# danbider/gp-quadrature

Hardware: AMD Instinct MI355X
Metric: GP-fits/sec (fit + posterior mean at the N training points), N=1e6 d=2 SE kernel (higher is better)
Workload: dtype f64; 1 GPU; 2D squared-exponential l=0.2 var=2 sigma2=0.2, eps=1e-4, global N=1e6 synthetic (BASELINE configs[1] at the metric's N=1e6), points sharded over the GPUs; n_per_gpu=1000000, global_n=1000000, d=2, mtot=23, M=529, mean_cg_iters=68, parallelism=points sharded over 1 GPU(s), CG replicated

## Files before the change

gp-quadrature_amd/csrc/cg_persistent.hip:

```cpp
#include <cmath>
#include <cstdlib>

#include "cg_plan_host.hpp"
#include "common.hpp"
#include "spectral_weights.hpp"
#include "toeplitz_cg.hpp"

namespace efgp {

namespace pcg {

constexpr int kRedWaves = kThreads / 64;

struct Pass {
    int dim;
    int n;
    int nstages;
    int radix[6];
    int w1_log2;
    int lines_log2;
    int other[2];
    int lo[2], hi[2];
    int in_limit;
    int out_lo, out_hi;
    int vs_pos, vs_c0, vs_c1;
    int pstride, s0, s1;
    int tw_lds;
    const double2* tw_glob;
};

struct Geom {
    int d;
    int n[3];
    int F[3];
    int ld[3];
    int M;
    int padded;
    int npass;
    Pass fwd[3];
    Pass inv[3];
    const double2* tw[3];
    int tw_lds_off[3];
    int tw_lds_total;
    int fuse_mid;
};

struct Args {
    Geom g;
    const double2* ws;
    const double* diag;
    const double* diag_scale;
    int b_times_ws;
    int zero_x0;
    const double2* x0;
    const double2* vhat;
    double sigmasq;
    int variant;
    double tol;
    int early_stop;
    int batched;
    int max_iter;
    const double2* b;
    double2* x;
    int* iters;
    double* hist;
    int hist_cap;
    int lz_steps;
    double* lz_alpha;
    double* lz_beta;
    double* lz_norm2;
    int wk_kind, wk_mtot;
    double wk_nu, wk_ell, wk_c0, wk_h;
    double2* ws_out;
    const double2* vsrc;
    int vL0, vL1;
    double2* vhat_out;
#ifdef EFGP_CG_STAMPS
    long long* stamps;
#endif
};

#ifdef EFGP_CG_STAMPS
#define EFGP_STAMP(slot)                                                     \
    do {                                                                     \
        if (blockIdx.x == 0 && threadIdx.x == 0) {                           \
            const long long now__ = (long long)__builtin_readcyclecounter(); \
            a.stamps[slot] += now__ - stamp_prev;                            \
            stamp_prev = now__;                                              \
        }                                                                    \
    } while (0)
#else
#define EFGP_STAMP(slot) \
    do {                 \
    } while (0)
#endif

__device__ __forceinline__ double2 cmulp(double2 a, double2 b) {
    return make_double2(a.x * b.x - a.y * b.y, a.x * b.y + a.y * b.x);
}
__device__ __forceinline__ double2 cadd(double2 a, double2 b) { return make_double2(a.x + b.x, a.y + b.y); }
__device__ __forceinline__ double2 csub(double2 a, double2 b) { return make_double2(a.x - b.x, a.y - b.y); }
__device__ __forceinline__ double2 mul_mi(double2 a) { return make_double2(a.y, -a.x); }

template <int R>
__device__ __forceinline__ void dft_fwd(double2 (&v)[R]);

template <>
__device__ __forceinline__ void dft_fwd<2>(double2 (&v)[2]) {
    double2 a = v[0], b = v[1];
    v[0] = cadd(a, b);
    v[1] = csub(a, b);
}

template <>
__device__ __forceinline__ void dft_fwd<4>(double2 (&v)[4]) {
    double2 t0 = cadd(v[0], v[2]), t1 = csub(v[0], v[2]);
    double2 t2 = cadd(v[1], v[3]), t3 = mul_mi(csub(v[1], v[3]));
    v[0] = cadd(t0, t2);
    v[1] = cadd(t1, t3);
    v[2] = csub(t0, t2);
    v[3] = csub(t1, t3);
}

template <>
__device__ __forceinline__ void dft_fwd<8>(double2 (&v)[8]) {
    double2 e[4] = {v[0], v[2], v[4], v[6]};
    double2 o[4] = {v[1], v[3], v[5], v[7]};
    dft_fwd<4>(e);
    dft_fwd<4>(o);
    const double h = 0.70710678118654752440;
    double2 o1 = make_double2(h * (o[1].x + o[1].y), h * (o[1].y - o[1].x));
    double2 o2 = mul_mi(o[2]);
    double2 o3 = make_double2(h * (o[3].y - o[3].x), -h * (o[3].x + o[3].y));
    v[0] = cadd(e[0], o[0]);
    v[4] = csub(e[0], o[0]);
    v[1] = cadd(e[1], o1);
    v[5] = csub(e[1], o1);
    v[2] = cadd(e[2], o2);
    v[6] = csub(e[2], o2);
    v[3] = cadd(e[3], o3);
    v[7] = csub(e[3], o3);
}

struct V8 {
    double2 a0, a1, a2, a3, a4, a5, a6, a7;
};
template <int T>
__device__ __forceinline__ double2& v8(V8& v) {
    if constexpr (T == 0) return v.a0;
    else if constexpr (T == 1) return v.a1;
    else if constexpr (T == 2) return v.a2;
    else if constexpr (T == 3) return v.a3;
    else if constexpr (T == 4) return v.a4;
    else if constexpr (T == 5) return v.a5;
    else if constexpr (T == 6) return v.a6;
    else return v.a7;
}
template <int T, int R>
__device__ __forceinline__ void spectral_mul_regs(double2 (&v)[R], V8& sp) {
    if constexpr (T < R) {
        double2 val = cmulp(v[T], v8<T>(sp));
        val.y = -val.y;
        v[T] = val;
        spectral_mul_regs<T + 1, R>(v, sp);
    }
}
template <int T, int R>
__device__ __forceinline__ void spectral_load_regs(V8& sp, const double2* __restrict__ vhat, int idx0, int step) {
    if constexpr (T < R) {
        v8<T>(sp) = vhat[idx0 + T * step];
        spectral_load_regs<T + 1, R>(sp, vhat, idx0, step);
    }
}

template <int R, bool INV, bool MID>
__device__ __forceinline__ void stage(const Geom& g, const Pass& p, int Ns, int ns_log2, bool first, bool last,
// ... 881 lines not shown
    if (!(asym <= 1e-16 * bb) || ws_bad != 0.0) {
#pragma unroll
        for (int s = 0; s < KS; ++s) {
            if (ok[s]) {
                a.x[base + idx[s]] = make_double2(__builtin_nan(""), __builtin_nan(""));
                a.x[base + (M - 1 - idx[s])] = make_double2(__builtin_nan(""), __builtin_nan(""));
            }
        }
        if (tid == 0) a.iters[row] = -2;
        return;
    }
    const double bn = sqrt(bb);
    const double den = bn > 0.0 ? bn : 1.0;
    const double den_eps = den + 1e-16, rcp_den = 1.0 / den_eps;
    if (wave == 3 && lane == 0) s_rcp = 1.0 / (rz + 1e-16);
    int it = 0;
    for (; it < a.max_iter;) {
        apply_A(pv, Ap);
        if (stop) break;
        double pAp = 0.0;
#pragma unroll
        for (int s = 0; s < KS; ++s) pAp += pv[s].x * Ap[s].x + pv[s].y * Ap[s].y;
        pAp = block_sum_h(pAp * wgt, red) + 1e-16;
        EFGP_STAMP(3);
        const double alpha = rz / pAp;
        double rr = 0.0, rzn = 0.0;
        double2 zv[KS];
#pragma unroll
        for (int s = 0; s < KS; ++s) {
            xv[s].x += alpha * pv[s].x;
            xv[s].y += alpha * pv[s].y;
            rv[s].x -= alpha * Ap[s].x;
            rv[s].y -= alpha * Ap[s].y;
            zv[s] = precond ? make_double2(div_rcp(rv[s].x, dg[s], rdg[s]), div_rcp(rv[s].y, dg[s], rdg[s])) : rv[s];
            rr += rv[s].x * rv[s].x + rv[s].y * rv[s].y;
            rzn += rv[s].x * zv[s].x + rv[s].y * zv[s].y;
        }
        rr *= wgt;
        rzn *= wgt;
        EFGP_STAMP(4);
        block_sum_pair_h(rr, rzn, red);
        EFGP_STAMP(5);
        ++it;
        if (wave == 3) {
            const double ratio = div_rcp(sqrt(rr), den_eps, rcp_den);
            const bool conv = a.early_stop && ((ratio < a.tol) || (a.batched && sqrt(rr) < 1e-12));
            if (lane == 0) {
                if (a.hist && row == 0 && it <= a.hist_cap) a.hist[it - 1] = ratio;
                s_stop = conv ? 1 : 0;
                s_rcp = 1.0 / (rzn + 1e-16);
            }
        }
        const double beta = div_rcp(rzn, rz + 1e-16, rcp_rz);
#pragma unroll
        for (int s = 0; s < KS; ++s) pv[s] = make_double2(zv[s].x + beta * pv[s].x, zv[s].y + beta * pv[s].y);
        rz = rzn;
    }
#pragma unroll
    for (int s = 0; s < KS; ++s) {
        if (ok[s]) {
            a.x[base + idx[s]] = xv[s];
            if (k0 > 0) a.x[base + (M - 1 - idx[s])] = s64::conjd(xv[s]);
        }
    }
    if (tid == 0) a.iters[row] = it;
}

namespace h48 {
constexpr int kThreadsH = 256, kWavesH = kThreadsH / 64;
constexpr int F = 48, HF = 24, NR = 12;
constexpr int LDR = 56;
constexpr int LT = 28;
constexpr int LX = 72;
constexpr int LQ = 82;
constexpr int G_ELEMS = NR * LDR, T_ELEMS = 2 * NR * LT, Q_ELEMS = HF * LQ;
static_assert(NR * LX <= Q_ELEMS, "the row lines' scratch aliases the column lines' scratch");
constexpr int kLdsElems = G_ELEMS + T_ELEMS + Q_ELEMS;
constexpr int ND = 4 * F;
constexpr int NC = 25;
constexpr int kReread = 8;
constexpr int LDV = 49;
constexpr int kLdsElemsDense = F * LDV + (kThreadsH / 8) * LX;
static_assert(2 * G_ELEMS + NR * LX <= kLdsElemsDense, "the iteration's G, Yh and row scratch alias the prologue's grid");

__device__ __forceinline__ void dft3(double2 b0, double2 b1, double2 b2, double2& x0, double2& x1, double2& x2) {
    const double s = 0.86602540378443864676;
    const double2 sm = cadd(b1, b2), df = csub(b1, b2);
    x0 = cadd(b0, sm);
    const double2 m = make_double2(fma(-0.5, sm.x, b0.x), fma(-0.5, sm.y, b0.y));
    x1 = make_double2(fma(s, df.y, m.x), fma(-s, df.x, m.y));
    x2 = make_double2(fma(-s, df.y, m.x), fma(s, df.x, m.y));
}
__device__ __forceinline__ void dft6(double2 (&v)[6]) {
    const double s = 0.86602540378443864676;
    double2 e0, e1, e2, o0, o1, o2;
    dft3(v[0], v[2], v[4], e0, e1, e2);
    dft3(v[1], v[3], v[5], o0, o1, o2);
    const double2 w1 = make_double2(fma(s, o1.y, 0.5 * o1.x), fma(-s, o1.x, 0.5 * o1.y));
    const double2 w2 = make_double2(fma(s, o2.y, -0.5 * o2.x), fma(-s, o2.x, -0.5 * o2.y));
    v[0] = cadd(e0, o0);
    v[3] = csub(e0, o0);
    v[1] = cadd(e1, w1);
    v[4] = csub(e1, w1);
    v[2] = cadd(e2, w2);
    v[5] = csub(e2, w2);
}
__device__ __forceinline__ void wave_sync() {
    __builtin_amdgcn_fence(__ATOMIC_ACQ_REL, "wavefront");
    __builtin_amdgcn_wave_barrier();
}
__device__ __forceinline__ void exchange_8to6(const double2 (&v)[8], double2 (&u)[6], bool writer, double2* __restrict__ wr,
                                              const double2* __restrict__ rd, const double2 (&tw)[5]) {
    wave_sync();
    if (writer) s64::store8_all<1>(wr, v);
    wave_sync();
#pragma unroll
    for (int t = 0; t < 6; ++t) u[t] = rd[9 * t];
#pragma unroll
    for (int t = 1; t < 6; ++t) u[t] = cmulp(u[t], tw[t - 1]);
    dft6(u);
}
__device__ __forceinline__ double exchange_8to6_norm(const double2 (&v)[8], double2 (&u)[6], bool writer, double2* __restrict__ wr,
                                                     const double2* __restrict__ rd, const double2 (&tw)[5], const double2 (&x)[4],
                                                     double scale) {
    wave_sync();
    if (writer) s64::store8_all<1>(wr, v);
    wave_sync();
#pragma unroll
    for (int t = 0; t < 6; ++t) u[t] = rd[9 * t];
    __builtin_amdgcn_sched_barrier(0);
    const double x01 = fma(x[0].x, x[0].x, x[0].y * x[0].y) + fma(x[1].x, x[1].x, x[1].y * x[1].y);
    const double x23 = fma(x[2].x, x[2].x, x[2].y * x[2].y) + fma(x[3].x, x[3].x, x[3].y * x[3].y);
    const double xx = scale * (x01 + x23);
    __builtin_amdgcn_sched_barrier(0);
#pragma unroll
    for (int t = 1; t < 6; ++t) u[t] = cmulp(u[t], tw[t - 1]);
    dft6(u);
    return xx;
}
__device__ __forceinline__ void exchange_6to8(double2 (&u)[6], double2 (&v)[8], double2* __restrict__ wr, const double2* __restrict__ rd,
                                              const double2 (&tw)[5]) {
#pragma unroll
    for (int t = 1; t < 6; ++t) u[t] = cmulp(u[t], tw[t - 1]);
    wave_sync();
#pragma unroll
    for (int t = 0; t < 6; ++t) wr[t] = u[t];
    wave_sync();
    s64::load8_all<9>(rd, v);
    h64::dft8_out4(v);
}

__device__ __forceinline__ double half_wave_sum(double v) {
    EFGP_DPP_ADD(v, 0x111, 0xF);
    EFGP_DPP_ADD(v, 0x112, 0xF);
    EFGP_DPP_ADD(v, 0x114, 0xF);
    EFGP_DPP_ADD(v, 0x118, 0xF);
    EFGP_DPP_ADD(v, 0x142, 0xA);
    const int lo = __builtin_amdgcn_readlane(__double2loint(v), 31);
    const int hi = __builtin_amdgcn_readlane(__double2hiint(v), 31);
    return __hiloint2double(hi, lo);
}

__device__ __forceinline__ double exchange_6to8_quot(double2 (&u)[6], double2 (&v)[8], double2* __restrict__ wr,
                                                     const double2* __restrict__ rd, const double2 (&tw)[5], double part, double num) {
#pragma unroll
    for (int t = 1; t < 6; ++t) u[t] = cmulp(u[t], tw[t - 1]);
// ... 56 lines not shown
        wave_sync();
#pragma unroll
        for (int t = 0; t < 6; ++t) wr[t] = u6[t];
        wave_sync();
        s64::load8_all<9>(rd, x8);
        dft_fwd<8>(x8);
        if (act && j < 6) {
#pragma unroll
            for (int t = 0; t < 8; ++t) buf[line * LD + j + 6 * t] = x8[t];
        }
    }
    __syncthreads();
#pragma unroll
    for (int ps = 0; ps < PASSES; ++ps) {
        const int line = slot + ps * SLOTS;
        const bool act = line < F;
#pragma unroll
        for (int t = 0; t < 6; ++t) u6[t] = act ? buf[(j + 8 * t) * LD + line] : make_double2(0.0, 0.0);
        dft6(u6);
#pragma unroll
        for (int t = 1; t < 6; ++t) u6[t] = cmulp(u6[t], tw[t - 1]);
        wave_sync();
#pragma unroll
        for (int t = 0; t < 6; ++t) wr[t] = u6[t];
        wave_sync();
        s64::load8_all<9>(rd, x8);
        dft_fwd<8>(x8);
        if (act && j < 6) {
#pragma unroll
            for (int t = 0; t < 8; ++t) {
                vhat[(j + 6 * t) * F + line] = x8[t];
                if (KEEP) buf[(j + 6 * t) * LD + line] = x8[t];
            }
        }
    }
}

template <int NT>
__device__ __forceinline__ void dense48_coeffs(double2* lds2, const double2 (&tw)[5], const double2* __restrict__ twg, int n,
                                               double2 (&cf)[NC]) {
    constexpr int SLOTS = NT / 8, PASSES = (F + SLOTS - 1) / SLOTS;
    double2* const buf = lds2;
    double2* const scr = lds2 + F * LDV;
    const int tid = threadIdx.x, slot = tid >> 3, j = tid & 7;
    double2* const wr = scr + slot * LX + 9 * j;
    const double2* const rd = scr + slot * LX + j;
    double2 u6[6], x8[8];
#pragma unroll
    for (int ps = 0; ps < PASSES; ++ps) {
        const int line = slot + ps * SLOTS;
        const bool act = line < F;
#pragma unroll
        for (int t = 0; t < 6; ++t) u6[t] = act ? s64::conjd(buf[(j + 8 * t) * LDV + line]) : make_double2(0.0, 0.0);
        dft6(u6);
#pragma unroll
        for (int t = 1; t < 6; ++t) u6[t] = cmulp(u6[t], tw[t - 1]);
        wave_sync();
#pragma unroll
        for (int t = 0; t < 6; ++t) wr[t] = u6[t];
        wave_sync();
        s64::load8_all<9>(rd, x8);
        dft_fwd<8>(x8);
        if (act && j < 6) {
#pragma unroll
            for (int t = 0; t < 8; ++t) buf[(j + 6 * t) * LDV + line] = s64::conjd(x8[t]);
        }
    }
    __syncthreads();
    const int f1 = tid % F, a0 = 3 * (tid / F);
    const bool dense = tid < ND;
    const double2 wc = twg[((n - 1) * f1) % F];
#pragma unroll
    for (int i = 0; i < NC; ++i) {
        const int l = a0 - 11 + i, al = l < 0 ? -l : l;
        double2 c = make_double2(0.0, 0.0);
        if (dense && al <= n - 1) {
            const double2 r = buf[(al + n - 1) * LDV + f1];
            c = make_double2(fma(r.y, wc.y, r.x * wc.x), fma(-r.x, wc.y, r.y * wc.x));
            if (l < 0) c.y = -c.y;
            if (l == 0) c.y = 0.0;
        }
        cf[i] = c;
    }
}
}

template <int VARIANT, bool FUSED = false, bool DENSE = true, bool FREQ_DOT = false>
__global__ __launch_bounds__(h48::kThreadsH) void cg_herm48_kernel(Args a) {
    using namespace h48;
    using h64::block_sum_h;
    using h64::block_sum_pair_h;
    using h64::dft8_in4;
    using h64::div_rcp;
    constexpr int KS = 4;
    static_assert(h64::kWavesH == kWavesH, "the block reductions are shared with the 64 x 64 kernel");
    static_assert(DENSE || !FREQ_DOT, "the row-frequency <p,Ap> reads what the per-frequency Toeplitz products hold");
    extern __shared__ double2 lds2[];
    __shared__ double red[4 * kWavesH];
    __shared__ double s_rcp;
    __shared__ int s_stop;
    __shared__ double s_part[FREQ_DOT ? ND + 8 * NR : 1];
    double2* const Gb = lds2;
    double2* const Tb = lds2 + G_ELEMS;
    double2* const Qb = Tb + (DENSE ? G_ELEMS : T_ELEMS);
    const int n = a.g.n[0], h = (n - 1) / 2, M = a.g.M;
    const int row = blockIdx.x;
    const int64_t base = (int64_t)row * M;
    const int tid = threadIdx.x, lane = tid & 63, wave = tid >> 6;
    const int k0 = tid >> 3, j = tid & 7;
    const bool row_role = tid < 8 * NR, vec_role = row_role && j < 6;
    const int jc = lane >> 3, ql = lane & 7, q = wave * 8 + ql;
    const bool col_role = wave < 3, col6 = jc < 6;
    const int k0s = row_role ? k0 : 0;
    double2* const xw = Qb + k0s * LX + 9 * j;
    const double2* const xr = Qb + k0s * LX + j;
    const int qs = col_role ? q : 0;
    double2* const qw = Qb + qs * LQ + 9 * jc;
    const double2* const qr = Qb + qs * LQ + jc;
    const bool dense_role = tid < ND;
    const int f1d = tid % F, kd = 3 * (tid / F);

    double2 twr[5], twc[5];
#pragma unroll
    for (int t = 1; t < 6; ++t) {
        twr[t - 1] = a.g.tw[0][j * t];
        twc[t - 1] = a.g.tw[0][jc * t];
    }
    if (FUSED) {
        vhat48_lines<kThreadsH, true>(a.vsrc, a.vL0, a.vL1, 1.0 / 2304.0, a.vhat_out, lds2);
        __syncthreads();
    }
    double sa[6], sb[6];
    double2 cf[DENSE ? NC : 1];
    if constexpr (DENSE) {
        if (!FUSED) {
#pragma unroll
            for (int k = 0; k < F * F / kThreadsH; ++k) {
                const int t = tid + k * kThreadsH, i0 = t / F, i1 = t - i0 * F;
                lds2[i0 * LDV + i1] = a.vhat[t];
            }
            __syncthreads();
        }
        dense48_coeffs<kThreadsH>(lds2, twr, a.g.tw[0], n, cf);
        __syncthreads();
    } else {
        const double2* const vh = FUSED ? lds2 : a.vhat;
        constexpr int LV = FUSED ? LDV : F;
#pragma unroll
        for (int t = 0; t < 6; ++t) {
            const int f0 = jc + 8 * t;
            const double2 va = vh[f0 * LV + qs], vb = vh[f0 * LV + qs + HF];
            const double2 wa = a.g.tw[0][((n - 1) * (f0 + qs)) % F], wb = a.g.tw[0][((n - 1) * (f0 + qs + HF)) % F];
            sa[t] = 0.5 * (va.x * wa.x + va.y * wa.y);
            sb[t] = -0.5 * (vb.x * wb.x + vb.y * wb.y);
        }
        if (FUSED) __syncthreads();
    }
    const bool z6_ok = jc > 0;
    const int jr = col6 ? jc : 0;

    double2 xv[KS], rv[KS], pv[KS];
    double wsr[KS], dg[KS], rdg[KS];
    bool ok[KS];
    int idx[KS];
    const bool precond = a.diag != nullptr || a.diag_scale != nullptr;
    const double wgt = k0 == 0 ? 1.0 : 2.0;
// ... 196 lines not shown
            rv[s] = csub(bv, Ap[s]);
            pv[s] = precond ? make_double2(div_rcp(rv[s].x, dg[s], rdg[s]), div_rcp(rv[s].y, dg[s], rdg[s])) : rv[s];
            rz += rv[s].x * pv[s].x + rv[s].y * pv[s].y;
            bb += bv.x * bv.x + bv.y * bv.y;
        }
    }
    rz *= wgt;
    bb *= wgt;
    block_sum_pair_h(rz, bb, red);
    asym = block_sum_h(asym, red);
    ws_bad = block_sum_h(ws_bad, red + kWavesH);
    if (!(asym <= 1e-16 * bb) || ws_bad != 0.0) {
#pragma unroll
        for (int s = 0; s < KS; ++s) {
            if (ok[s]) {
                a.x[base + idx[s]] = make_double2(__builtin_nan(""), __builtin_nan(""));
                a.x[base + (M - 1 - idx[s])] = make_double2(__builtin_nan(""), __builtin_nan(""));
            }
        }
        if (tid == 0) a.iters[row] = -2;
        return;
    }
    const double bn = sqrt(bb);
    const double den = bn > 0.0 ? bn : 1.0;
    const double den_eps = den + 1e-16, rcp_den = 1.0 / den_eps;
    if (wave == 3 && lane == 0) s_rcp = 1.0 / (rz + 1e-16);
    int it = 0;
    for (; it < a.max_iter;) {
        apply_A(pv, Ap);
        if (stop) break;
        double alpha;
        if constexpr (FREQ_DOT) {
            alpha = alpha_fd;
        } else {
            double pAp = 0.0;
#pragma unroll
            for (int s = 0; s < KS; ++s) pAp += pv[s].x * Ap[s].x + pv[s].y * Ap[s].y;
            pAp = block_sum_h(pAp * wgt, red) + 1e-16;
            EFGP_STAMP(3);
            alpha = rz / pAp;
        }
        double rr = 0.0, rzn = 0.0;
        double2 zv[KS];
#pragma unroll
        for (int s = 0; s < KS; ++s) {
            xv[s].x += alpha * pv[s].x;
            xv[s].y += alpha * pv[s].y;
            rv[s].x -= alpha * Ap[s].x;
            rv[s].y -= alpha * Ap[s].y;
            zv[s] = precond ? make_double2(div_rcp(rv[s].x, dg[s], rdg[s]), div_rcp(rv[s].y, dg[s], rdg[s])) : rv[s];
            rr += rv[s].x * rv[s].x + rv[s].y * rv[s].y;
            rzn += rv[s].x * zv[s].x + rv[s].y * zv[s].y;
        }
        rr *= wgt;
        rzn *= wgt;
        EFGP_STAMP(4);
        block_sum_pair_h(rr, rzn, red);
        EFGP_STAMP(5);
        ++it;
        if (wave == 3) {
            const double ratio = div_rcp(sqrt(rr), den_eps, rcp_den);
            const bool conv = a.early_stop && ((ratio < a.tol) || (a.batched && sqrt(rr) < 1e-12));
            if (lane == 0) {
                if (a.hist && row == 0 && it <= a.hist_cap) a.hist[it - 1] = ratio;
                s_stop = conv ? 1 : 0;
                s_rcp = 1.0 / (rzn + 1e-16);
            }
        }
        const double beta = div_rcp(rzn, rz + 1e-16, rcp_rz);
#pragma unroll
        for (int s = 0; s < KS; ++s) pv[s] = make_double2(zv[s].x + beta * pv[s].x, zv[s].y + beta * pv[s].y);
        rz = rzn;
    }
#pragma unroll
    for (int s = 0; s < KS; ++s) {
        if (ok[s]) {
            a.x[base + idx[s]] = xv[s];
            if (k0 > 0) a.x[base + (M - 1 - idx[s])] = s64::conjd(xv[s]);
        }
    }
    if (tid == 0) a.iters[row] = it;
}

namespace l1d {
__device__ __forceinline__ void wave_sync() {
    __builtin_amdgcn_fence(__ATOMIC_ACQ_REL, "wavefront");
    __builtin_amdgcn_wave_barrier();
}
__device__ __forceinline__ double2* wave_fft(double2* x, double2* y, int F, int lg, const double2* __restrict__ tw) {
    const int lane = threadIdx.x;
    int Ns = 1, rem = lg;
    while (rem >= 2) {
        const int nb = F >> 2, tstep = F / (Ns * 4);
        for (int j = lane; j < nb; j += 64) {
            const int k = j & (Ns - 1), j0 = ((j - k) << 2) + k;
            double2 v0 = x[j], v1 = x[j + nb], v2 = x[j + 2 * nb], v3 = x[j + 3 * nb];
            if (k != 0) {
                v1 = cmulp(v1, tw[k * tstep]);
                v2 = cmulp(v2, tw[2 * k * tstep]);
                v3 = cmulp(v3, tw[3 * k * tstep]);
            }
            const double2 t0 = cadd(v0, v2), t1 = csub(v0, v2), t2 = cadd(v1, v3), d13 = csub(v1, v3);
            const double2 t3 = make_double2(d13.y, -d13.x);
            y[j0] = cadd(t0, t2);
            y[j0 + Ns] = cadd(t1, t3);
            y[j0 + 2 * Ns] = csub(t0, t2);
            y[j0 + 3 * Ns] = csub(t1, t3);
        }
        wave_sync();
        double2* t = x;
        x = y;
        y = t;
        Ns <<= 2;
        rem -= 2;
    }
    if (rem == 1) {
        const int nb = F >> 1;
        for (int j = lane; j < nb; j += 64) {
            const int k = j & (Ns - 1), j0 = ((j - k) << 1) + k;
            const double2 v0 = x[j];
            double2 v1 = x[j + nb];
            if (k != 0) v1 = cmulp(v1, tw[k]);
            y[j0] = cadd(v0, v1);
            y[j0 + Ns] = csub(v0, v1);
        }
        wave_sync();
        double2* t = x;
        x = y;
        y = t;
    }
    return x;
}
}

__global__ __launch_bounds__(64) void cg_line1d_kernel(Args a) {
    using namespace l1d;
    extern __shared__ double2 lds2[];
    const int F = a.g.F[0], n = a.g.n[0], M = a.g.M;
    const int lg = 31 - __clz(F);
    double2* const X = lds2;
    double2* const Y = lds2 + F;
    double2* const TW = Y + F;
    double2* const VH = TW + F;
    const int lane = threadIdx.x, row = blockIdx.x;
    const int64_t base = (int64_t)row * M;
    for (int q = lane; q < F; q += 64) {
        TW[q] = a.g.tw[0][q];
        VH[q] = a.vhat[q];
    }
    double2 xv[KS], rv[KS], pv[KS], wsv[KS];
    double dg[KS];
    const bool precond = a.diag != nullptr || a.diag_scale != nullptr;
#pragma unroll
    for (int s = 0; s < KS; ++s) {
        const int t = lane + 64 * s;
        if (t < M) {
            xv[s] = a.zero_x0 ? make_double2(0.0, 0.0) : a.x0[base + t];
            wsv[s] = a.ws[t];
            dg[s] = jacobi_entry(a, wsv[s], t);
        } else {
            xv[s] = wsv[s] = make_double2(0.0, 0.0);
            dg[s] = 1.0;
        }
        rv[s] = pv[s] = make_double2(0.0, 0.0);
    }
    wave_sync();
// ... 539 lines not shown
        g.F[i] = i < tg.d ? (int)tg.F[i] : 1;
        g.tw[i] = i < tg.d ? twiddles[i] : nullptr;
    }
    int stride = 1;
    for (int i = 2; i >= 0; --i) {
        if (i >= tg.d) {
            g.ld[i] = 0;
            continue;
        }
        g.ld[i] = stride;
        stride *= (i == tg.d - 1 && tg.d > 1) ? g.F[i] + 1 : g.F[i];
    }
    g.padded = stride;
    g.M = (int)tg.M;
    g.npass = tg.d;
    for (int q = 0; q < tg.d; ++q) {
        set_pass(g, tg.d - 1 - q, false, g.fwd[q]);
        Pass& p = g.inv[q];
        set_pass(g, q, true, p);
        for (int i = 0; i < p.nstages / 2; ++i) std::swap(p.radix[i], p.radix[p.nstages - 1 - i]);
    }
    order_lines(g);
    g.fuse_mid = 1;
    place_twiddles_and_strides(g);
}

static void solve_args(const CgSolve& s, const double2* vhat, int* d_iters, const LanczosOut* lz, Args& a) {
    a.ws_out = nullptr;
    a.vsrc = nullptr;
    a.vhat_out = nullptr;
    a.ws = s.ws;
    a.diag = s.diag;
    a.diag_scale = s.diag_scale;
    a.b_times_ws = s.b_times_ws;
    a.zero_x0 = s.zero_x0;
    a.x0 = s.x0 ? s.x0 : s.x;
    a.vhat = vhat;
    a.sigmasq = s.sigmasq;
    a.variant = s.variant;
    a.tol = s.tol;
    a.early_stop = s.early_stop;
    a.batched = s.batched;
    a.max_iter = s.max_iter;
    a.b = s.b;
    a.x = s.x;
    a.iters = d_iters;
    a.hist = cg_history().buf;
    a.hist_cap = cg_history().capacity;
    a.lz_steps = lz ? lz->steps : 0;
    a.lz_alpha = lz ? lz->alpha : nullptr;
    a.lz_beta = lz ? lz->beta : nullptr;
    a.lz_norm2 = lz ? lz->norm2 : nullptr;
}

static void operands48(const Herm48Operands& h48, const MeanFusedOperands* fuse, Args& a) {
    a.vhat = fuse ? nullptr : h48.vhat;
    a.g.F[0] = a.g.F[1] = 48;
    a.g.tw[0] = a.g.tw[1] = h48.tw;
    if (!fuse) return;
    a.ws = nullptr;
    a.wk_kind = fuse->kind;
    a.wk_mtot = fuse->mtot;
    a.wk_nu = fuse->nu;
    a.wk_ell = fuse->ell;
    a.wk_c0 = fuse->c0;
    a.wk_h = fuse->h;
    a.ws_out = fuse->ws_out;
    a.vsrc = fuse->v;
    a.vL0 = fuse->L0;
    a.vL1 = fuse->L1;
    a.vhat_out = fuse->vhat48_out;
}

struct PickLaunch {
    void (*kernel)(Args);
    int threads;
    size_t lds;
    const char* what;
};
static PickLaunch launch_of(const PersistentChoice& c, int variant, const Geom& g) {
    constexpr size_t lds48d = (size_t)h48::kLdsElemsDense * sizeof(double2);
    static_assert(h48::kLdsElemsDense >= h48::kLdsElems, "the fused prologue's LDS covers the iteration's");
    const bool freq_dot = std::getenv("EFGP_CG48_MODE_DOT") == nullptr;
    switch (c.pick) {
        case PersistentPick::fused48: {
            void (*const dense[2])(Args) = {cg_herm48_kernel<0, true, true, false>, cg_herm48_kernel<0, true, true, true>};
            return {c.dense48 ? dense[freq_dot] : cg_herm48_kernel<0, true, false>, h48::kThreadsH, lds48d, "fused mean solve (48x48)"};
        }
        case PersistentPick::herm48: {
            void (*const dense[2][2])(Args) = {{cg_herm48_kernel<0, false, true, false>, cg_herm48_kernel<1, false, true, false>},
                                               {cg_herm48_kernel<0, false, true, true>, cg_herm48_kernel<1, false, true, true>}};
            void (*const fft2d[2])(Args) = {cg_herm48_kernel<0, false, false>, cg_herm48_kernel<1, false, false>};
            return {(c.dense48 ? dense[freq_dot] : fft2d)[variant != 0], h48::kThreadsH,
                    c.dense48 ? lds48d : (size_t)h48::kLdsElems * sizeof(double2), "persistent CG (48x48, Hermitian)"};
        }
        case PersistentPick::herm64:
            return {variant == 0 ? cg_herm64_kernel<0> : cg_herm64_kernel<1>, h64::kThreadsH, (size_t)h64::kLdsElems * sizeof(double2),
                    "persistent CG (64x64, Hermitian)"};
        case PersistentPick::line1d:
            return {cg_line1d_kernel, 64, (size_t)4 * g.F[0] * sizeof(double2), "persistent CG (1-D)"};
        case PersistentPick::fast64:
            return {cg_persistent_2d64_kernel, kThreads, (size_t)2 * 64 * 72 * sizeof(double2), "persistent CG (64x64)"};
        case PersistentPick::generic:
            break;
    }
    return {cg_persistent_kernel, kThreads, ((size_t)2 * g.padded + g.tw_lds_total) * sizeof(double2), "persistent CG"};
}

}

int persistent_cg_launch(const ToepGeom& full, const double2* const* tw_full, const double2* vhat, const Herm48Operands* h48,
                         const CgSolve& s, int* d_iters, hipStream_t stream, const LanczosOut* lz, const MeanFusedOperands* fuse) {
    using namespace pcg;
    ToepGeom tg;
    const double2* twiddles[3] = {nullptr, nullptr, nullptr};
    if (squeeze_unit_axes(full, tw_full, &tg, twiddles) == 0) {
        set_error("persistent CG: a grid of a single cell has no transform to run");
        return EFGP_EUNSUPPORTED;
    }
    Args a;
    pass_geometry(tg, twiddles, a.g);
    solve_args(s, vhat, d_iters, lz, a);
#ifdef EFGP_CG_STAMPS
    {
        static long long* d_stamps = nullptr;
        if (!d_stamps) (void)hipMalloc((void**)&d_stamps, 16 * sizeof(long long));
        (void)hipMemsetAsync(d_stamps, 0, 16 * sizeof(long long), stream);
        a.stamps = d_stamps;
        g_last_stamps = d_stamps;
    }
#endif
    PersistentChoice c;
    if (const int rc = pick_persistent(full, s, h48 != nullptr && h48->vhat != nullptr, lz != nullptr, fuse != nullptr, &c)) return rc;
    if (c.pick == PersistentPick::fused48 || c.pick == PersistentPick::herm48) operands48(*h48, fuse, a);
    const PickLaunch l = launch_of(c, s.variant, a.g);
    if (const int rc = raise_dynamic_lds((const void*)l.kernel, l.lds, l.what)) return rc;
    {
        KernelTimer timer("cg_solve", stream);
        hipLaunchKernelGGL(l.kernel, dim3(s.nbatch), dim3(l.threads), l.lds, stream, a);
    }
    const hipError_t e = hipGetLastError();
    if (e != hipSuccess) {
        set_error("persistent CG launch failed: %s", hipGetErrorString(e));
        return EFGP_EHIP;
    }
    return EFGP_OK;
}

}
```

Baseline: 4456 GP fits/s of the global N=1e6 problem (whole job; the points are sharded over the GPUs).

## Add eight-wave 48x48 persistent CG kernel with dedicated Toeplitz-product waves

Adds a 512-thread persistent CG kernel for the 48x48 Hermitian dense path. Two waves run the per-row FFT and vector updates, while six waves each hold precomputed symmetric/antisymmetric lag coefficient pairs and compute one or two Toeplitz frequency products per thread. It is selected by default when the dense, frequency-dot path is active. The aim is to spread the dense Toeplitz matvec across more waves and halve the FMA count through symmetric coefficient pairing, at the cost of larger blocks, higher register pressure and more block-wide barriers per iteration.

```diff
diff --git a/gp-quadrature_amd/csrc/cg_persistent.hip b/gp-quadrature_amd/csrc/cg_persistent.hip
--- a/gp-quadrature_amd/csrc/cg_persistent.hip
+++ b/gp-quadrature_amd/csrc/cg_persistent.hip
@@ -89,9 +89,27 @@
             stamp_prev = now__;                                              \
         }                                                                    \
     } while (0)
+#define EFGP_STAMP_BY(slot, who)                                             \
+    do {                                                                     \
+        if (blockIdx.x == 0 && threadIdx.x == (who)) {                       \
+            const long long now__ = (long long)__builtin_readcyclecounter(); \
+            a.stamps[slot] += now__ - stamp_prev;                            \
+            stamp_prev = now__;                                              \
+        }                                                                    \
+    } while (0)
+#define EFGP_STAMP_RESTART(who)                                                                                  \
+    do {                                                                                                         \
+        if (blockIdx.x == 0 && threadIdx.x == (who)) stamp_prev = (long long)__builtin_readcyclecounter();       \
+    } while (0)
 #else
 #define EFGP_STAMP(slot) \
     do {                 \
+    } while (0)
+#define EFGP_STAMP_BY(slot, who) \
+    do {                         \
+    } while (0)
+#define EFGP_STAMP_RESTART(who) \
+    do {                        \
     } while (0)
 #endif
 
@@ -1139,6 +1157,10 @@
 constexpr int LDV = 49;
 constexpr int kLdsElemsDense = F * LDV + (kThreadsH / 8) * LX;
 static_assert(2 * G_ELEMS + NR * LX <= kLdsElemsDense, "the iteration's G, Yh and row scratch alias the prologue's grid");
+constexpr int kThreadsP = 512, kRowWavesP = 2, kPairWavesP = 3;
+constexpr int NDP = kThreadsP - 64 * kRowWavesP;
+static_assert(NDP == 8 * F && 64 * kPairWavesP == 4 * F, "no wave mixes two-row and one-row groups");
+constexpr int kLdsElemsPairs = F * LDV + (kThreadsP / 8) * LX;
 
 __device__ __forceinline__ void dft3(double2 b0, double2 b1, double2 b2, double2& x0, double2& x1, double2& x2) {
     const double s = 0.86602540378443864676;
@@ -1361,6 +1383,74 @@
         }
         cf[i] = c;
     }
+}
+
+template <int NT>
+__device__ __forceinline__ void dense48_inverse_pass(double2* lds2, const double2 (&tw)[5]) {
+    constexpr int SLOTS = NT / 8, PASSES = (F + SLOTS - 1) / SLOTS;
+    double2* const buf = lds2;
+    double2* const scr = lds2 + F * LDV;
+    const int tid = threadIdx.x, slot = tid >> 3, j = tid & 7;
+    double2* const wr = scr + slot * LX + 9 * j;
+    const double2* const rd = scr + slot * LX + j;
+    double2 u6[6], x8[8];
+#pragma unroll
+    for (int ps = 0; ps < PASSES; ++ps) {
+        const int line = slot + ps * SLOTS;
+        const bool act = line < F;
+#pragma unroll
+        for (int t = 0; t < 6; ++t) u6[t] = act ? s64::conjd(buf[(j + 8 * t) * LDV + line]) : make_double2(0.0, 0.0);
+        dft6(u6);
+#pragma unroll
+        for (int t = 1; t < 6; ++t) u6[t] = cmulp(u6[t], tw[t - 1]);
+        wave_sync();
+#pragma unroll
+        for (int t = 0; t < 6; ++t) wr[t] = u6[t];
+        wave_sync();
+        s64::load8_all<9>(rd, x8);
+        dft_fwd<8>(x8);
+        if (act && j < 6) {
+#pragma unroll
+            for (int t = 0; t < 8; ++t) buf[(j + 6 * t) * LDV + line] = s64::conjd(x8[t]);
+        }
+    }
+}
+__device__ __forceinline__ double2 lag_coeff(const double2* buf, double2 wc, int n, int f1, int l) {
+    const int al = l < 0 ? -l : l;
+    double2 c = make_double2(0.0, 0.0);
+    if (al <= n - 1) {
+        const double2 r = buf[(al + n - 1) * LDV + f1];
+        c = make_double2(fma(r.y, wc.y, r.x * wc.x), fma(-r.x, wc.y, r.y * wc.x));
+        if (l < 0) c.y = -c.y;
+        if (l == 0) c.y = 0.0;
+    }
+    return c;
+}
+
+constexpr int NM = NR - 1;
+struct PairCoeffs {
+    double2 c0;
+    double2 S[NM], Q[NM];
+};
+__device__ __forceinline__ void pair_coeffs(const double2* buf, double2 wc, int n, int f1, int k0, PairCoeffs& pc) {
+    pc.c0 = lag_coeff(buf, wc, n, f1, k0);
+#pragma unroll
+    for (int m = 1; m < NR; ++m) {
+        const double2 cm = lag_coeff(buf, wc, n, f1, k0 - m), cp = lag_coeff(buf, wc, n, f1, k0 + m);
+        pc.S[m - 1] = cadd(cm, cp);
+        pc.Q[m - 1] = csub(cm, cp);
+    }
+}
+__device__ __forceinline__ double2 pair_product(const PairCoeffs& pc, const double2 (&gm)[NR]) {
+    double2 acc = make_double2(pc.c0.x * gm[0].x, pc.c0.y * gm[0].x);
+#pragma unroll
+    for (int m = 1; m < NR; ++m) {
+        acc.x = fma(pc.S[m - 1].x, gm[m].x, acc.x);
+        acc.y = fma(pc.S[m - 1].y, gm[m].x, acc.y);
+        acc.x = fma(-pc.Q[m - 1].y, gm[m].y, acc.x);
+        acc.y = fma(pc.Q[m - 1].x, gm[m].y, acc.y);
+    }
+    return acc;
 }
 }
 
@@ -1723,6 +1813,316 @@
     if (tid == 0) a.iters[row] = it;
 }
 
+template <int NOUT>
+__device__ __forceinline__ void pairs_dense_role(const Args& a, double2* lds2, double* red, double* s_part, double* s_rcp, int* s_stop) {
+    using namespace h48;
+    using h64::div_rcp;
+    const double2* const Gb = lds2;
+    double2* const Tb = lds2 + G_ELEMS;
+    const int n = a.g.n[0];
+    const int tid = threadIdx.x, lane = tid & 63, d = tid - 64 * kRowWavesP;
+    const int f1d = d % F, grp = d / F, kd = NOUT == 2 ? 2 * grp : grp + 4;
+    const bool duty = tid >= kThreadsP - 64;
+    PairCoeffs pc[NOUT];
+    {
+        const double2 wc = a.g.tw[0][((n - 1) * f1d) % F];
+#pragma unroll
+        for (int o = 0; o < NOUT; ++o) pair_coeffs(lds2, wc, n, f1d, kd + o, pc[o]);
+    }
+    __syncthreads();
+#ifdef EFGP_CG_STAMPS
+    long long stamp_prev = 0;
+#endif
+    const double2* const g0 = Gb + f1d;
+    double2* const t0 = Tb + kd * LDR + f1d;
+    auto products = [&]() __attribute__((always_inline)) -> bool {
+        __syncthreads();
+        if (*s_stop) return false;
+        EFGP_STAMP_RESTART(64 * kRowWavesP);
+        double2 gm[NR], acc[NOUT], gk[NOUT];
+#pragma unroll
+        for (int m = 0; m < NR; ++m) gm[m] = g0[m * LDR];
+#pragma unroll
+        for (int o = 0; o < NOUT; ++o) acc[o] = pair_product(pc[o], gm);
+#pragma unroll
+        for (int o = 0; o < NOUT; ++o) gk[o] = g0[(kd + o) * LDR];
+        t0[0] = make_double2(acc[0].x, kd == 0 ? 0.0 : -acc[0].y);
+        if constexpr (NOUT == 2) t0[LDR] = make_double2(acc[1].x, -acc[1].y);
+        EFGP_STAMP_BY(1, 64 * kRowWavesP);
+        const double t0r = kd == 0 ? gk[0].x * acc[0].x : 2.0 * fma(gk[0].y, acc[0].y, gk[0].x * acc[0].x);
+        if constexpr (NOUT == 2) s_part[d] = fma(2.0, fma(gk[1].y, acc[1].y, gk[1].x * acc[1].x), t0r);
+        else s_part[d] = t0r;
+        __syncthreads();
+        EFGP_STAMP_BY(6, 64 * kRowWavesP);
+        return true;
+    };
+    if (!a.zero_x0) products();
+    __syncthreads();
+    const double rz = red[0] + red[4], bb = red[1] + red[5], asym = red[2] + red[6], ws_bad = red[3] + red[7];
+    if (!(asym <= 1e-16 * bb) || ws_bad != 0.0) return;
+    const double bn = sqrt(bb);
+    const double den = bn > 0.0 ? bn : 1.0;
+    const double den_eps = den + 1e-16, rcp_den = 1.0 / den_eps;
+    if (duty && lane == 0) *s_rcp = 1.0 / (rz + 1e-16);
+    for (int it = 0; it < a.max_iter;) {
+        if (!products()) break;
+        __syncthreads();
+        ++it;
+        if (duty) {
+            const double rr = red[0] + red[1], rzn = red[2] + red[3];
+            const double ratio = div_rcp(sqrt(rr), den_eps, rcp_den);
+            const bool conv = a.early_stop && ((ratio < a.tol) || (a.batched && sqrt(rr) < 1e-12));
+            if (lane == 0) {
+                if (a.hist && blockIdx.x == 0 && it <= a.hist_cap) a.hist[it - 1] = ratio;
+                *s_stop = conv ? 1 : 0;
+                *s_rcp = 1.0 / (rzn + 1e-16);
+            }
+        }
+    }
+}
+
+template <int VARIANT, bool FUSED = false>
+__global__ __launch_bounds__(h48::kThreadsP) void cg_herm48_pairs_kernel(Args a) {
+    using namespace h48;
+    using h64::dft8_in4;
+    using h64::div_rcp;
+    constexpr int KS = 4;
+    extern __shared__ double2 lds2[];
+    __shared__ double red[4 * kRowWavesP];
+    __shared__ double s_rcp;
+    __shared__ int s_stop;
+    __shared__ double s_part[NDP + 8 * NR];
+    double2* const Gb = lds2;
+    double2* const Tb = lds2 + G_ELEMS;
+    double2* const Qb = Tb + G_ELEMS;
+    const int n = a.g.n[0], h = (n - 1) / 2, M = a.g.M;
+    const int row = blockIdx.x;
+    const int64_t base = (int64_t)row * M;
+    const int tid = threadIdx.x, lane = tid & 63;
+    const int wave = __builtin_amdgcn_readfirstlane(tid >> 6);
+    const int k0 = tid >> 3, j = tid & 7;
+
+    double2 twr[5];
+#pragma unroll
+    for (int t = 1; t < 6; ++t) twr[t - 1] = a.g.tw[0][j * t];
+    if (tid == 0) {
+        s_stop = 0;
+        s_rcp = 0.0;
+    }
+    if (FUSED) {
+        vhat48_lines<kThreadsP, true>(a.vsrc, a.vL0, a.vL1, 1.0 / 2304.0, a.vhat_out, lds2);
+    } else {
+#pragma unroll
+        for (int k = 0; k < (F * F + kThreadsP - 1) / kThreadsP; ++k) {
+            const int t = tid + k * kThreadsP, i0 = t / F, i1 = t - i0 * F;
+            if (t < F * F) lds2[i0 * LDV + i1] = a.vhat[t];
+        }
+    }
+    __syncthreads();
+    dense48_inverse_pass<kThreadsP>(lds2, twr);
+    __syncthreads();
+    if (wave >= kRowWavesP + kPairWavesP) {
+        pairs_dense_role<1>(a, lds2, red, s_part, &s_rcp, &s_stop);
+        return;
+    }
+    if (wave >= kRowWavesP) {
+        pairs_dense_role<2>(a, lds2, red, s_part, &s_rcp, &s_stop);
+        return;
+    }
+
+    const bool row_role = tid < 8 * NR, vec_role = row_role && j < 6;
+    const int k0s = row_role ? k0 : 0;
+    double2* const xw = Qb + k0s * LX + 9 * j;
+    const double2* const xr = Qb + k0s * LX + j;
+    double2 xv[KS], rv[KS], pv[KS];
+    double wsr[KS], dg[KS], rdg[KS];
+    bool ok[KS];
+    int idx[KS];
+    const bool precond = a.diag != nullptr || a.diag_scale != nullptr;
+    const double wgt = k0 == 0 ? 1.0 : 2.0;
+    double ws_bad = 0.0;
+#pragma unroll
+    for (int s = 0; s < KS; ++s) {
+        const int k1 = s == 0 ? j : (s == 1 ? j + 6 : (s == 2 ? j - 12 : j - 6));
+        ok[s] = vec_role && k0 <= h && k1 <= h && -k1 <= h;
+        idx[s] = ok[s] ? (k0 + h) * n + (k1 + h) : 0;
+        double ws_im = 0.0;
+        if (ok[s] && FUSED) {
+            xv[s] = make_double2(0.0, 0.0);
+            const double2 w = make_double2(spectral_weight_at(a.wk_kind, a.g.d, a.wk_nu, a.wk_ell, a.wk_c0, a.wk_h, a.wk_mtot, idx[s]), 0.0);
+            a.ws_out[idx[s]] = w;
+            a.ws_out[M - 1 - idx[s]] = w;
+            wsr[s] = w.x;
+            dg[s] = jacobi_entry(a, w, idx[s]);
+        } else if (ok[s]) {
+            xv[s] = a.zero_x0 ? make_double2(0.0, 0.0) : a.x0[base + idx[s]];
+            const double2 w = a.ws[idx[s]], wm = a.ws[M - 1 - idx[s]];
+            wsr[s] = w.x;
+            ws_im = w.y * w.y + (w.x - wm.x) * (w.x - wm.x) + wm.y * wm.y;
+            dg[s] = jacobi_entry(a, w, idx[s]);
+        } else {
+            xv[s] = make_double2(0.0, 0.0);
+            wsr[s] = 0.0;
+            dg[s] = 1.0;
+        }
+        ws_bad += ws_im;
+        rdg[s] = 1.0 / dg[s];
+        rv[s] = pv[s] = make_double2(0.0, 0.0);
+    }
+    __syncthreads();
+
+#ifdef EFGP_CG_STAMPS
+    long long stamp_prev = (long long)__builtin_readcyclecounter();
+#endif
+    int stop = 0;
+    double rcp_rz = 0.0;
+    double rz = 0.0;
+    double alpha_fd = 0.0;
+    auto apply_A = [&](const double2 (&u)[KS], double2 (&Au)[KS]) __attribute__((always_inline)) {
+        double2 v[8], u6[6];
+        EFGP_STAMP(7);
+        if (row_role) {
+            dft8_in4(make_double2(wsr[0] * u[0].x, wsr[0] * u[0].y), make_double2(wsr[1] * u[1].x, wsr[1] * u[1].y),
+                     make_double2(wsr[2] * u[2].x, wsr[2] * u[2].y), make_double2(wsr[3] * u[3].x, wsr[3] * u[3].y), v);
+            const double uu = exchange_8to6_norm(v, u6, j < 6, xw, xr, twr, u, VARIANT == 0 ? wgt * a.sigmasq : wgt);
+            double2* g0 = Gb + k0 * LDR + j;
+#pragma unroll
+            for (int t = 0; t < 6; ++t) g0[8 * t] = u6[t];
+            s_part[NDP + tid] = uu;
+        }
+        __syncthreads();
+        stop = s_stop;
+        rcp_rz = s_rcp;
+        if (stop) return;
+        EFGP_STAMP(0);
+        __syncthreads();
+        EFGP_STAMP_RESTART(0);
+        if (row_role) {
+            double pt[15];
+            const double* sp = s_part + (lane & 31);
+#pragma unroll
+            for (int t = 0; t < 15; ++t) pt[t] = sp[32 * t];
+            const double2* tp = Tb + k0 * LDR + j;
+#pragma unroll
+            for (int t = 0; t < 6; ++t) u6[t] = tp[8 * t];
+            __builtin_amdgcn_sched_barrier(0);
+            double tsum = (((pt[0] + pt[1]) + (pt[2] + pt[3])) + ((pt[4] + pt[5]) + (pt[6] + pt[7]))) + ((pt[8] + pt[9]) + (pt[10] + pt[11]));
+            if (VARIANT == 1) tsum /= a.sigmasq;
+            const double uAu = tsum + ((pt[12] + pt[13]) + pt[14]);
+            dft6(u6);
+            alpha_fd = exchange_6to8_quot(u6, v, xw, xr, twr, uAu, rz);
+            const double2 y[KS] = {s64::conjd(v[0]), s64::conjd(v[1]), s64::conjd(v[6]), s64::conjd(v[7])};
+#pragma unroll
+            for (int s = 0; s < KS; ++s) {
+                const double2 gg = make_double2(wsr[s] * y[s].x, wsr[s] * y[s].y);
+                double2 val;
+                if (VARIANT == 0) val = make_double2(gg.x + a.sigmasq * u[s].x, gg.y + a.sigmasq * u[s].y);
+                else val = make_double2(gg.x / a.sigmasq + u[s].x, gg.y / a.sigmasq + u[s].y);
+                Au[s] = ok[s] ? val : make_double2(0.0, 0.0);
+            }
+        } else {
+            alpha_fd = 0.0;
+#pragma unroll
+            for (int s = 0; s < KS; ++s) Au[s] = make_double2(0.0, 0.0);
+        }
+        EFGP_STAMP(2);
+    };
+
+    double2 Ap[KS];
+    if (a.zero_x0) {
+#pragma unroll
+        for (int s = 0; s < KS; ++s) Ap[s] = make_double2(0.0, 0.0);
+    } else {
+        apply_A(xv, Ap);
+    }
+    double bb = 0.0, asym = 0.0;
+#pragma unroll
+    for (int s = 0; s < KS; ++s) {
+        if (ok[s]) {
+            double2 bv = a.b[base + idx[s]];
+            double2 bm = a.b[base + (M - 1 - idx[s])];
+            if (a.b_times_ws) {
+                bv = make_double2(wsr[s] * bv.x, wsr[s] * bv.y);
+                bm = make_double2(wsr[s] * bm.x, wsr[s] * bm.y);
+            }
+            asym += (bv.x - bm.x) * (bv.x - bm.x) + (bv.y + bm.y) * (bv.y + bm.y);
+            rv[s] = csub(bv, Ap[s]);
+            pv[s] = precond ? make_double2(div_rcp(rv[s].x, dg[s], rdg[s]), div_rcp(rv[s].y, dg[s], rdg[s])) : rv[s];
+            rz += rv[s].x * pv[s].x + rv[s].y * pv[s].y;
+            bb += bv.x * bv.x + bv.y * bv.y;
+        }
+    }
+    rz = wave_sum(rz * wgt);
+    bb = wave_sum(bb * wgt);
+    asym = wave_sum(asym);
+    ws_bad = wave_sum(ws_bad);
+    if (lane == 0) {
+        red[4 * wave] = rz;
+        red[4 * wave + 1] = bb;
+        red[4 * wave + 2] = asym;
+        red[4 * wave + 3] = ws_bad;
+    }
+    __syncthreads();
+    rz = red[0] + red[4];
+    bb = red[1] + red[5];
+    asym = red[2] + red[6];
+    ws_bad = red[3] + red[7];
+    if (!(asym <= 1e-16 * bb) || ws_bad != 0.0) {
+#pragma unroll
+        for (int s = 0; s < KS; ++s) {
+            if (ok[s]) {
+                a.x[base + idx[s]] = make_double2(__builtin_nan(""), __builtin_nan(""));
+                a.x[base + (M - 1 - idx[s])] = make_double2(__builtin_nan(""), __builtin_nan(""));
+            }
+        }
+        if (tid == 0) a.iters[row] = -2;
+        return;
+    }
+    int it = 0;
+    for (; it < a.max_iter;) {
+        apply_A(pv, Ap);
+        if (stop) break;
+        const double alpha = alpha_fd;
+        double rr = 0.0, rzn = 0.0;
+        double2 zv[KS];
+#pragma unroll
+        for (int s = 0; s < KS; ++s) {
+            xv[s].x += alpha * pv[s].x;
+            xv[s].y += alpha * pv[s].y;
+            rv[s].x -= alpha * Ap[s].x;
+            rv[s].y -= alpha * Ap[s].y;
+            zv[s] = precond ? make_double2(div_rcp(rv[s].x, dg[s], rdg[s]), div_rcp(rv[s].y, dg[s], rdg[s])) : rv[s];
+            rr += rv[s].x * rv[s].x + rv[s].y * rv[s].y;
+            rzn += rv[s].x * zv[s].x + rv[s].y * zv[s].y;
+        }
+        rr *= wgt;
+        rzn *= wgt;
+        EFGP_STAMP(4);
+        rr = wave_sum(rr);
+        rzn = wave_sum(rzn);
+        if (lane == 0) {
+            red[wave] = rr;
+            red[2 + wave] = rzn;
+        }
+        __syncthreads();
+        rzn = red[2] + red[3];
+        EFGP_STAMP(5);
+        ++it;
+        const double beta = div_rcp(rzn, rz + 1e-16, rcp_rz);
+#pragma unroll
+        for (int s = 0; s < KS; ++s) pv[s] = make_double2(zv[s].x + beta * pv[s].x, zv[s].y + beta * pv[s].y);
+        rz = rzn;
+    }
+#pragma unroll
+    for (int s = 0; s < KS; ++s) {
+        if (ok[s]) {
+            a.x[base + idx[s]] = xv[s];
+            if (k0 > 0) a.x[base + (M - 1 - idx[s])] = s64::conjd(xv[s]);
+        }
+    }
+    if (tid == 0) a.iters[row] = it;
+}
+
 namespace l1d {
 __device__ __forceinline__ void wave_sync() {
     __builtin_amdgcn_fence(__ATOMIC_ACQ_REL, "wavefront");
@@ -2428,12 +2828,18 @@
     constexpr size_t lds48d = (size_t)h48::kLdsElemsDense * sizeof(double2);
     static_assert(h48::kLdsElemsDense >= h48::kLdsElems, "the fused prologue's LDS covers the iteration's");
     const bool freq_dot = std::getenv("EFGP_CG48_MODE_DOT") == nullptr;
+    const bool pairs = c.dense48 && freq_dot && std::getenv("EFGP_CG48_LAG_COEFFS") == nullptr;
+    constexpr size_t lds48p = (size_t)h48::kLdsElemsPairs * sizeof(double2);
     switch (c.pick) {
         case PersistentPick::fused48: {
+            if (pairs) return {cg_herm48_pairs_kernel<0, true>, h48::kThreadsP, lds48p, "fused mean solve (48x48, eight waves)"};
             void (*const dense[2])(Args) = {cg_herm48_kernel<0, true, true, false>, cg_herm48_kernel<0, true, true, true>};
             return {c.dense48 ? dense[freq_dot] : cg_herm48_kernel<0, true, false>, h48::kThreadsH, lds48d, "fused mean solve (48x48)"};
         }
         case PersistentPick::herm48: {
+            if (pairs)
+                return {variant == 0 ? cg_herm48_pairs_kernel<0> : cg_herm48_pairs_kernel<1>, h48::kThreadsP, lds48p,
+                        "persistent CG (48x48, Hermitian, eight waves)"};
             void (*const dense[2][2])(Args) = {{cg_herm48_kernel<0, false, true, false>, cg_herm48_kernel<1, false, true, false>},
                                                {cg_herm48_kernel<0, false, true, true>, cg_herm48_kernel<1, false, true, true>}};
             void (*const fft2d[2])(Args) = {cg_herm48_kernel<0, false, false>, cg_herm48_kernel<1, false, false>};
```

Measured after the change: 4859 GP fits/s of the global N=1e6 problem (whole job; the points are sharded over the GPUs) (median of 6 runs). 9.0% higher.
